# PoseLib/PoseLib

Measured on AMD Instinct MI355X. Metric: scored RANSAC hypotheses/sec (P3P@5k corrs, 5pt@5k corrs), higher is better.
Workload: dtype f64; 1 GPU; p3p_5000; correspondences=5000, problems_in_flight_per_gpu=128, distinct_scenes=64

## Files before the change

poselib_amd/csrc/kernels.hip:

```cpp
#include "pl_kernels.h"
#include "pl_global.h"
#include "pl_lm_chain.inc"
#include "pl_device.h"
#include <atomic>
#include "pl_prefilter.h"
#include <cstdlib>
#include "pl_sampler.h"
#include "pl_solver_h4.h"
#include "pl_solver_p3p.h"
#include "pl_solver_p5lp_radial.h"
#include "pl_solver_rel.h"

namespace pl {

typedef const float __attribute__((address_space(4))) *uniform_f32_ptr;
typedef const double __attribute__((address_space(4))) *uniform_f64_ptr;
typedef const uint32_t __attribute__((address_space(4))) *uniform_u32_ptr;
__device__ __forceinline__ uniform_f32_ptr as_uniform(const float *p) { return (uniform_f32_ptr)(uintptr_t)p; }
__device__ __forceinline__ uniform_f64_ptr as_uniform(const double *p) { return (uniform_f64_ptr)(uintptr_t)p; }
__device__ __forceinline__ uniform_u32_ptr as_uniform(const uint32_t *p) { return (uniform_u32_ptr)(uintptr_t)p; }

__device__ __forceinline__ double wave_sum(double v) {
#pragma unroll
    for (int off = 32; off > 0; off >>= 1)
// ... 840 lines not shown
                                                   const uint32_t *__restrict__ num_hyp_ptr, uint32_t hyp_capacity, double thr2,
                                                   const PrefilterArgs &pf, uint32_t *__restrict__ part_count,
                                                   double *__restrict__ part_score, uint32_t slice, uint32_t chunk,
                                                   uint32_t nslices) {
    constexpr int kWaves = kQueueThreads / 64;
    constexpr int ND = 5, P = kRadialP, NPW = kRadialChunk;
    __shared__ double s_pts[ND][NPW];
    __shared__ uint16_t s_queue[kWaves][kQueueCap];
    __shared__ double s_acc_s[kWaves][64];
    __shared__ uint32_t s_acc_c[kWaves][64];
    constexpr int kInlierCap = 128;
    __shared__ double s_inl_v[kWaves][kInlierCap];
    __shared__ uint16_t s_inl_g[kWaves][kInlierCap];
    __shared__ uint32_t s_next_unit;
    const int lane = threadIdx.x & 63;
    const int wave = __builtin_amdgcn_readfirstlane((int)(threadIdx.x >> 6));

    float pf32[P][ND];
    float bnd[P][2];
    uint64_t vmask[P];
    const float thrp = pf_radial1d_thr(pf.thr);
#pragma unroll
    for (int p = 0; p < P; ++p) {
        const uint32_t i = chunk * NPW + p * 64 + lane;
        const bool valid = i < pts.n;
        const uint32_t ic = valid ? i : 0u;
        vmask[p] = __builtin_amdgcn_ballot_w64(valid);
        double x[ND];
        load_point<EST_RAD1D>(pts, ic, x);
        if (wave == p) {
#pragma unroll
            for (int d = 0; d < ND; ++d)
                s_pts[d][p * 64 + lane] = x[d];
        }
        pf_radial1d_point(x, pf.thr, pf32[p], bnd[p]);
    }
    if (threadIdx.x == 0)
        s_next_unit = 0;
    __syncthreads();

    const uint32_t H = *as_uniform(num_hyp_ptr);
    const uniform_f32_ptr sh = as_uniform(shadow);
    uint16_t *const queue = s_queue[wave];
    double *const acc_s = s_acc_s[wave];
    uint32_t *const acc_c = s_acc_c[wave];
    double *const inl_v = s_inl_v[wave];
    uint16_t *const inl_g = s_inl_g[wave];

    const uint32_t waves_per_chunk = nslices * kWaves;
    auto request_ticket = [&]() -> uint32_t {
        uint32_t t = 0;
        if (lane == 0) {
            const uint32_t k = atomicAdd(&s_next_unit, 1u);
            t = slice * kWaves + (k % kWaves) + (k / kWaves) * waves_per_chunk;
        }
        return t;
    };
    uint32_t ticket = (uint32_t)__builtin_amdgcn_readfirstlane((int)request_ticket());
    uint32_t kb, gn;
    while (unit_of_ticket(ticket, H, waves_per_chunk, kb, gn)) {
        const uint32_t pending = request_ticket();
        acc_s[lane] = 0.0;
        acc_c[lane] = 0;
        uint32_t qhead = 0, qtail = 0;
        uint32_t ihead = 0, itail = 0;

        auto add_inliers = [&](uint32_t n) {
            __builtin_amdgcn_fence(__ATOMIC_ACQ_REL, "wavefront");
            const bool act = (uint32_t)lane < n;
            const uint32_t at = (ihead + lane) & (kInlierCap - 1);
            const uint32_t g = act ? (uint32_t)inl_g[at] : 0x7fu;
            const double v = act ? inl_v[at] : 0.0;
            const uint64_t actmask = __builtin_amdgcn_ballot_w64(act);
            const uint32_t g0 = (uint32_t)__builtin_amdgcn_readfirstlane((int)g);
            if (!__builtin_amdgcn_ballot_w64(act && g != g0)) {
                const double tot = wave_sum_dpp(v);
                if (lane == 0) {
                    acc_s[g0] += tot;
                    acc_c[g0] += (uint32_t)__popcll(actmask);
                }
            } else {
                add_run_totals(v, actmask, g, act, lane, acc_s, acc_c);
            }
            ihead += n;
        };

        auto drain = [&](uint32_t n) {
            __builtin_amdgcn_fence(__ATOMIC_ACQ_REL, "wavefront");
            const bool act = (uint32_t)lane < n;
            const uint32_t e = act ? (uint32_t)queue[(qhead + lane) & (kQueueCap - 1)] : 0xffffu;
            const uint32_t g = e >> 9, pi = act ? (e & 0x1ffu) : 0u;
            double x[ND];
#pragma unroll
            for (int d = 0; d < ND; ++d)
                x[d] = s_pts[d][pi];
            const double *Mp = compact64 + (size_t)(kb + (act ? g : 0u)) * kModelDoubles;
            double M[kModelDoubles];
#pragma unroll
            for (int i = 0; i < kModelDoubles; ++i)
                M[i] = Mp[i];
            double r2;
            const bool in = radial1d_inlier(M, x[0], x[1], x[2], x[3], x[4], thr2, r2) && act;
            const uint64_t inmask = __builtin_amdgcn_ballot_w64(in);
            if (inmask) {
                const uint32_t below = __builtin_amdgcn_mbcnt_hi((uint32_t)(inmask >> 32), __builtin_amdgcn_mbcnt_lo((uint32_t)inmask, 0u));
                if (in) {
                    inl_v[(itail + below) & (kInlierCap - 1)] = r2;
                    inl_g[(itail + below) & (kInlierCap - 1)] = (uint16_t)g;
                }
                itail += (uint32_t)__popcll(inmask);
                if (itail - ihead >= 64u)
                    add_inliers(64u);
            }
            qhead += n;
        };

        auto step = [&](const float(&r)[15], uint32_t g) {
            if ((r[0] != r[0]) | (r[1] != r[1]) | (r[2] != r[2]) | (r[3] != r[3]) | (r[4] != r[4]) | (r[5] != r[5]) | (r[9] != r[9]) | (r[10] != r[10]))
                return;
            uint64_t m[P];
            uint64_t any = 0;
            if (!pf.enabled || !(r[14] < __builtin_huge_valf())) {
#pragma unroll
                for (int p = 0; p < P; ++p)
                    m[p] = vmask[p], any |= m[p];
            } else {
#pragma unroll
                for (int p = 0; p < P; ++p) {
                    m[p] = vmask[p] & ~__builtin_amdgcn_ballot_w64(pf_radial1d_outlier(r, thrp, pf32[p], bnd[p]));
                    any |= m[p];
                }
            }
            if (any) {
#pragma unroll
                for (int p = 0; p < P; ++p) {
                    if (m[p]) {
                        const uint32_t below = __builtin_amdgcn_mbcnt_hi((uint32_t)(m[p] >> 32),
                                                                         __builtin_amdgcn_mbcnt_lo((uint32_t)m[p], 0u));
                        if ((m[p] >> lane) & 1u)
                            queue[(qtail + below) & (kQueueCap - 1)] = (uint16_t)((g << 9) | (uint32_t)(p * 64 + lane));
                        qtail += (uint32_t)__popcll(m[p]);
                    }
                }
                while (qtail - qhead >= 64u)
                    drain(64u);
            }
        };
        auto fetch = [&](float(&r)[15], uint32_t g) {
            const uniform_f32_ptr sp = sh + (size_t)(kb + g) * 16;
#pragma unroll
            for (int i = 0; i < 15; ++i)
                r[i] = sp[i];
        };

        float ra[15], rb[15];
        fetch(ra, 0);
        for (uint32_t g = 0; g < gn; g += 2) {
            const bool two = g + 1 < gn;
            if (two)
                fetch(rb, g + 1);
            step(ra, g);
            if (two) {
                if (g + 2 < gn)
                    fetch(ra, g + 2);
                step(rb, g + 1);
            }
        }
        while (qtail != qhead)
            drain(min(64u, qtail - qhead));
        if (itail != ihead)
            add_inliers(itail - ihead);
        __builtin_amdgcn_fence(__ATOMIC_ACQ_REL, "wavefront");
        if ((uint32_t)lane < gn) {
            const size_t o = (size_t)chunk * hyp_capacity + kb + lane;
            part_score[o] = acc_s[lane];
            part_count[o] = acc_c[lane];
        }
        ticket = (uint32_t)__builtin_amdgcn_readfirstlane((int)pending);
    }
}
__global__ __launch_bounds__(kQueueThreads) void k_score_radial1d(PointSet pts, const float *__restrict__ shadow,
                                                                  const double *__restrict__ compact64,
                                                                  const uint32_t *__restrict__ num_hyp_ptr, uint32_t hyp_capacity,
                                                                  double thr2, PrefilterArgs pf, uint32_t *__restrict__ part_count,
                                                                  double *__restrict__ part_score) {
    score_radial1d_body(pts, shadow, compact64, num_hyp_ptr, hyp_capacity, thr2, pf, part_count, part_score, blockIdx.x, blockIdx.y,
                       gridDim.x);
}

typedef _Float16 half4_t __attribute__((ext_vector_type(4)));
typedef _Float16 half8_t __attribute__((ext_vector_type(8)));
typedef float float16_t __attribute__((ext_vector_type(16)));
constexpr int kMfmaThreads = 512;

__device__ __forceinline__ bool slice_chunk_of_workgroup(uint32_t slices, uint32_t chunks, uint32_t &slice, uint32_t &chunk) {
    const uint32_t T = slices * chunks, L = blockIdx.x + gridDim.x * blockIdx.y;
    if (L >= T)
        return false;
    const uint32_t x = L & 7u, p = x * (T >> 3) + min(x, T & 7u) + (L >> 3);
    slice = p / chunks;
    chunk = p - slice * chunks;
    return true;
}

constexpr int kMfmaQueueCap = 1024;
template <int EST>
__device__ __forceinline__ void mfma_drain(const uint16_t *queue, uint32_t first, uint32_t n0, uint32_t n1, const double *pts, int npw,
                                       const double *__restrict__ models, uint32_t unit_slots, double thr2, double *acc_s,
                                       uint32_t *acc_c) {
    const int lane = threadIdx.x & 63;
    struct Batch {
        uint32_t g;
        bool act;
        double x[EST == EST_ABS ? 5 : 4];
        double M[kModelDoubles];
    };
    auto fetch = [&](uint32_t n, uint32_t at, Batch &b) {
        b.act = (uint32_t)lane < n;
        const uint32_t e = b.act ? (uint32_t)queue[(at + lane) & (kMfmaQueueCap - 1)] : 0xffffu;
        const uint32_t pi = b.act ? (e & 0x1ffu) : 0u;
        b.g = e >> 9;
#pragma unroll
        for (int d = 0; d < (EST == EST_ABS ? 5 : 4); ++d)
            b.x[d] = pts[d * npw + pi];
        const uint32_t slot_g = (uint32_t)__shfl((int)unit_slots, (int)(b.act ? b.g : 0u), 64);
        const double *Mp = models + (size_t)slot_g * kModelStride;
#pragma unroll
        for (int i = 0; i < kModelDoubles; ++i)
            b.M[i] = Mp[i];
    };
    auto finish = [&](const Batch &b) {
        double r2;
        const bool in = eval_point<EST>(b.M, b.x, thr2, r2) && b.act;
        const double v = in ? r2 : 0.0;
        const uint64_t inmask = __builtin_amdgcn_ballot_w64(in);
        const uint32_t g0 = (uint32_t)__builtin_amdgcn_readfirstlane((int)b.g);
        if (inmask && !__builtin_amdgcn_ballot_w64(b.act && b.g != g0)) {
            const double tot = wave_sum_dpp(v);
            if (lane == 0) {
                acc_s[g0] += tot;
                acc_c[g0] += (uint32_t)__popcll(inmask);
            }
        } else if (inmask) {
            add_run_totals(v, inmask, b.g, b.act, lane, acc_s, acc_c);
        }
    };
    __builtin_amdgcn_fence(__ATOMIC_ACQ_REL, "wavefront");
    Batch b0, b1;
    fetch(n0, first, b0);
    if (n1) {
        fetch(n1, first + n0, b1);
        finish(b0);
        finish(b1);
    } else {
        finish(b0);
    }
}

template <int PG>
__device__ __forceinline__ void abs16_tile_bits(const half8_t (&Aop)[kAbs16Dirs], const uint4 (&s_b)[1 + kAbs16Dirs][PG][32], int col, int half,
                                                uint32_t (&out)[16]) {
#pragma unroll
    for (int v = 0; v < 16; ++v)
        out[v] = 0u;
    const float16_t kZero = {0, 0, 0, 0, 0, 0, 0, 0, 0, 0, 0, 0, 0, 0, 0, 0};
    auto products = [&](int g, float16_t &D0, float16_t &D1, float16_t &D2) {
        half8_t Bop[kAbs16Dirs];
#pragma unroll
        for (int d = 0; d < kAbs16Dirs; ++d) {
            const uint4 braw = s_b[half ? 1 + d : 0][g][col];
            __builtin_memcpy(&Bop[d], &braw, 16);
        }
        D0 = __builtin_amdgcn_mfma_f32_32x32x16_f16(Aop[0], Bop[0], kZero, 0, 0, 0);
        D1 = __builtin_amdgcn_mfma_f32_32x32x16_f16(Aop[1], Bop[1], kZero, 0, 0, 0);
        D2 = __builtin_amdgcn_mfma_f32_32x32x16_f16(Aop[2], Bop[2], kZero, 0, 0, 0);
    };
    float16_t D0, D1, D2;
    products(0, D0, D1, D2);
#pragma unroll 16
    for (int g = 1; g < PG; ++g) {
        uint32_t T[16];
#pragma unroll
        for (int v = 0; v < 16; ++v)
            T[v] = __float_as_uint(D0[v]) | __float_as_uint(D1[v]) | __float_as_uint(D2[v]);
        products(g, D0, D1, D2);
#pragma unroll
        for (int v = 0; v < 16; ++v)
            out[v] = __builtin_amdgcn_alignbit(out[v], T[v], 31);
        __builtin_amdgcn_sched_group_barrier(0x002, 16, 0);
        __builtin_amdgcn_sched_group_barrier(0x100, 3, 0);
        __builtin_amdgcn_sched_group_barrier(0x002, 4, 0);
        __builtin_amdgcn_sched_group_barrier(0x008, 1, 0);
        __builtin_amdgcn_sched_group_barrier(0x002, 4, 0);
        __builtin_amdgcn_sched_group_barrier(0x008, 1, 0);
        __builtin_amdgcn_sched_group_barrier(0x002, 4, 0);
        __builtin_amdgcn_sched_group_barrier(0x008, 1, 0);
        __builtin_amdgcn_sched_group_barrier(0x002, 4, 0);
    }
#pragma unroll
    for (int v = 0; v < 16; ++v) {
        const uint32_t sg = __float_as_uint(D0[v]) | __float_as_uint(D1[v]) | __float_as_uint(D2[v]);
        out[v] = __builtin_amdgcn_alignbit(out[v], sg, 31);
    }
}

constexpr int kScoreAll = 0, kScoreLead = 1, kScoreSel = 2, kScoreCount = 3, kScoreCountAll = 4;
template <int PG, int MODE = kScoreAll>
__device__ __forceinline__ void score_mfma_body(const PointSet &pts, const uint4 *__restrict__ shadow16,
                                                const uint4 *__restrict__ points16,
                                                const double *__restrict__ models, const uint32_t *__restrict__ slots,
                                                const uint32_t *__restrict__ num_hyp_ptr, uint32_t hyp_capacity,
                                                double thr2, uint32_t *__restrict__ part_count,
                                                double *__restrict__ part_score, uint32_t slice, uint32_t chunk,
                                                uint32_t nslices, const uint32_t *__restrict__ sel = nullptr,
                                                uint32_t lead = 0) {
    constexpr int kWaves = kMfmaThreads / 64;
    constexpr int NPW = 32 * PG;
    __shared__ double s_pts[5][NPW];
    __shared__ uint16_t s_queue[kWaves][kMfmaQueueCap];
    __shared__ double s_acc_s[kWaves][64];
    __shared__ uint32_t s_acc_c[kWaves][64];
    __shared__ uint32_t s_next_unit;
    __shared__ uint4 s_b[1 + kAbs16Dirs][PG][32];
    const int lane = threadIdx.x & 63;
    const int wave = __builtin_amdgcn_readfirstlane((int)(threadIdx.x >> 6));
    const int col = lane & 31, half = lane >> 5;

    const uint32_t H = MODE == kScoreLead ? min(*as_uniform(num_hyp_ptr), lead) : *as_uniform(num_hyp_ptr);
    const uint32_t waves_per_chunk = nslices * kWaves;
    {
        uint32_t kb0, gn0;
        if (!unit_of_ticket<32u>(slice * kWaves, H, waves_per_chunk, kb0, gn0))
            return;
    }

    uint32_t validbits = 0;
#pragma unroll
    for (int g = 0; g < PG; ++g)
        validbits |= (chunk * NPW + g * 32 + col < pts.n) ? (1u << (PG - 1 - g)) : 0u;
    const uint4 *const prow = points16 + (size_t)chunk * NPW * 4;
    for (uint32_t j = threadIdx.x; j < (uint32_t)NPW; j += kMfmaThreads) {
        const uint32_t i = chunk * NPW + j;
        const uint32_t ic = i < pts.n ? i : 0u;
#pragma unroll
        for (int d = 0; d < 5; ++d)
            s_pts[d][j] = pts.a[d][ic];
#pragma unroll
        for (int r = 0; r < 1 + kAbs16Dirs; ++r)
            s_b[r][j >> 5][j & 31] = prow[(size_t)j * 4 + r];
    }
    if (threadIdx.x == 0)
        s_next_unit = 0;
    __syncthreads();

    uint16_t *const queue = s_queue[wave];
    double *const acc_s = s_acc_s[wave];
    uint32_t *const acc_c = s_acc_c[wave];
    auto request_ticket = [&]() -> uint32_t {
        uint32_t t = 0;
        if (lane == 0) {
            const uint32_t k = atomicAdd(&s_next_unit, 1u);
            t = slice * kWaves + (k % kWaves) + (k / kWaves) * waves_per_chunk;
        }
        return t;
    };
    uint32_t ticket = (uint32_t)__builtin_amdgcn_readfirstlane((int)request_ticket());
    uint32_t kb, gn;
    while (unit_of_ticket<32u>(ticket, H, waves_per_chunk, kb, gn)) {
        const uint32_t pending = request_ticket();
        uint32_t unit_pos = 0;
        if constexpr (MODE == kScoreSel)
            unit_pos = sel ? sel[kb + min((uint32_t)lane, gn - 1u)] : kb + min((uint32_t)lane, gn - 1u);
        const uint32_t unit_slots = slots[MODE == kScoreSel ? unit_pos : kb + min((uint32_t)lane, gn - 1u)];
        acc_s[lane] = 0.0;
        acc_c[lane] = 0;
        uint32_t qhead = 0, qtail = 0;

        auto drain_pair = [&](uint32_t n2) {
            mfma_drain<EST_ABS>(queue, qhead, 64u, n2, &s_pts[0][0], NPW, models, unit_slots, thr2, acc_s, acc_c);
            qhead += 64u + n2;
        };
        auto drain = [&](uint32_t n) {
            mfma_drain<EST_ABS>(queue, qhead, n, 0u, &s_pts[0][0], NPW, models, unit_slots, thr2, acc_s, acc_c);
            qhead += n;
        };

        const uint32_t ngroups32 = (gn + 31u) / 32u;
        auto load_a = [&](uint32_t hg, uint4 (&A)[kAbs16Dirs]) {
            const uint4 *row = shadow16 + (size_t)(kb + 32u * hg + (uint32_t)col) * 4;
            if constexpr (MODE == kScoreSel)
                row = shadow16 + (size_t)(uint32_t)__shfl((int)unit_pos, (int)(32u * hg + (uint32_t)col), 64) * 4;
#pragma unroll
            for (int d = 0; d < kAbs16Dirs; ++d)
                A[d] = row[half ? 3 : d];
        };
        uint4 Araw[kAbs16Dirs];
        load_a(0, Araw);
        for (uint32_t hg = 0; hg < ngroups32; ++hg) {
            half8_t Aop[kAbs16Dirs];
#pragma unroll
            for (int d = 0; d < kAbs16Dirs; ++d)
                __builtin_memcpy(&Aop[d], &Araw[d], 16);
            if (hg + 1 < ngroups32)
                load_a(hg + 1, Araw);
            uint32_t out[16];
            abs16_tile_bits<PG>(Aop, s_b, col, half, out);
            const bool partial_group = hg * 32u + 32u > gn;
            auto expand_round = [&](int v, bool check_slot) {
                const uint32_t slot = hg * 32u + 8u * (uint32_t)(v >> 2) + 4u * (uint32_t)half + (uint32_t)(v & 3);
                uint32_t bits = ~out[v] & validbits;
                if (check_slot && slot >= gn)
                    bits = 0u;
                const uint64_t anyb = __builtin_amdgcn_ballot_w64(bits != 0u);
                if (anyb) {
                    const uint32_t cnt = (uint32_t)__popc(bits);
                    if (!__builtin_amdgcn_ballot_w64(cnt > 1u)) {
                        const uint32_t below = __builtin_amdgcn_mbcnt_hi((uint32_t)(anyb >> 32), __builtin_amdgcn_mbcnt_lo((uint32_t)anyb, 0u));
                        if (bits) {
                            const uint32_t g = (uint32_t)(PG - 1 - (31 - __clz((int)bits)));
                            queue[(qtail + below) & (kMfmaQueueCap - 1)] = (uint16_t)((slot << 9) | (g * 32u + (uint32_t)col));
                        }
                        qtail += (uint32_t)__popcll(anyb);
                    } else {
                        const uint32_t incl = wave_scan_u32(cnt);
                        const uint32_t total = (uint32_t)__builtin_amdgcn_readlane((int)incl, 63);
                        uint32_t pos = qtail + incl - cnt;
                        uint32_t rest = bits;
                        while (rest) {
                            const int hi = 31 - __clz((int)rest);
                            rest &= ~(1u << hi);
                            const uint32_t g = (uint32_t)(PG - 1 - hi);
                            queue[pos & (kMfmaQueueCap - 1)] = (uint16_t)((slot << 9) | (g * 32u + (uint32_t)col));
                            ++pos;
                        }
                        qtail += total;
                    }
                    while (qtail - qhead >= 128u)
                        drain_pair(64u);
                }
            };
            if (partial_group) {
#pragma unroll
                for (int v = 0; v < 16; ++v)
                    expand_round(v, true);
            } else {
#pragma unroll
                for (int v = 0; v < 16; ++v)
                    expand_round(v, false);
            }
        }
        if (qtail - qhead > 64u)
            drain_pair(qtail - qhead - 64u);
        else if (qtail != qhead)
            drain(qtail - qhead);
        __builtin_amdgcn_fence(__ATOMIC_ACQ_REL, "wavefront");
        if ((uint32_t)lane < gn) {
            const size_t o = MODE == kScoreSel ? (size_t)chunk * hyp_capacity + unit_pos : (size_t)chunk * hyp_capacity + kb + lane;
            part_score[o] = acc_s[lane];
            part_count[o] = acc_c[lane];
        }
        ticket = (uint32_t)__builtin_amdgcn_readfirstlane((int)pending);
    }
}

template <int PG>
__device__ __forceinline__ void score_count_body(uint32_t n_points, const uint4 *__restrict__ shadow16, const uint4 *__restrict__ points16,
                                                 const uint32_t *__restrict__ num_hyp_ptr, uint32_t hyp_capacity,
                                                 uint32_t *__restrict__ survivors, uint32_t slice, uint32_t chunk, uint32_t nslices,
                                                 uint32_t first) {
    constexpr int kWaves = kMfmaThreads / 64;
    constexpr int NPW = 32 * PG;
    __shared__ uint4 s_b[1 + kAbs16Dirs][PG][32];
    __shared__ uint32_t s_cnt[kWaves][64];
    __shared__ uint32_t s_next_unit;
    const int lane = threadIdx.x & 63;
    const int wave = __builtin_amdgcn_readfirstlane((int)(threadIdx.x >> 6));
    const int col = lane & 31, half = lane >> 5;
    const uint32_t Hall = *as_uniform(num_hyp_ptr);
    if (Hall <= first)
        return;
    const uint32_t H = Hall - first;
    const uint32_t waves_per_chunk = nslices * kWaves;
    {
        uint32_t kb0, gn0;
        if (!unit_of_ticket<32u>(slice * kWaves, H, waves_per_chunk, kb0, gn0))
            return;
    }
    uint32_t validbits = 0;
#pragma unroll
    for (int g = 0; g < PG; ++g)
        validbits |= (chunk * NPW + g * 32 + col < n_points) ? (1u << (PG - 1 - g)) : 0u;
    const uint4 *const prow = points16 + (size_t)chunk * NPW * 4;
    for (uint32_t j = threadIdx.x; j < (uint32_t)NPW; j += kMfmaThreads) {
#pragma unroll
        for (int r = 0; r < 1 + kAbs16Dirs; ++r)
            s_b[r][j >> 5][j & 31] = prow[(size_t)j * 4 + r];
    }
    if (threadIdx.x == 0)
        s_next_unit = 0;
    __syncthreads();

    uint32_t *const cnt = s_cnt[wave];
    auto request_ticket = [&]() -> uint32_t {
        uint32_t t = 0;
        if (lane == 0) {
            const uint32_t k = atomicAdd(&s_next_unit, 1u);
            t = slice * kWaves + (k % kWaves) + (k / kWaves) * waves_per_chunk;
        }
        return t;
    };
    uint32_t ticket = (uint32_t)__builtin_amdgcn_readfirstlane((int)request_ticket());
    uint32_t kb, gn;
    while (unit_of_ticket<32u>(ticket, H, waves_per_chunk, kb, gn)) {
        const uint32_t pending = request_ticket();
        const uint32_t ngroups32 = (gn + 31u) / 32u;
        auto load_a = [&](uint32_t hg, uint4 (&A)[kAbs16Dirs]) {
            const uint4 *row = shadow16 + (size_t)min(first + kb + 32u * hg + (uint32_t)col, Hall - 1u) * 4;
#pragma unroll
            for (int d = 0; d < kAbs16Dirs; ++d)
                A[d] = row[half ? 3 : d];
        };
        uint4 Araw[kAbs16Dirs];
        load_a(0, Araw);
        for (uint32_t hg = 0; hg < ngroups32; ++hg) {
            half8_t Aop[kAbs16Dirs];
#pragma unroll
            for (int d = 0; d < kAbs16Dirs; ++d)
                __builtin_memcpy(&Aop[d], &Araw[d], 16);
            if (hg + 1 < ngroups32)
                load_a(hg + 1, Araw);
            uint32_t out[16];
            abs16_tile_bits<PG>(Aop, s_b, col, half, out);
            uint32_t pk[6] = {0u, 0u, 0u, 0u, 0u, 0u};
#pragma unroll
            for (int v = 0; v < 16; ++v)
                pk[v / 3] += (uint32_t)__popc(~out[v] & validbits) << (10 * (v % 3));
#pragma unroll
            for (int j = 0; j < 6; ++j) {
                uint32_t s = pk[j];
                s += dpp_shift_u32<0x111>(s);
                s += dpp_shift_u32<0x112>(s);
                s += dpp_shift_u32<0x114>(s);
                s += dpp_shift_u32<0x118>(s);
                s += dpp_shift_u32<0x142, 0xa>(s);
                pk[j] = s;
            }
            if (col == 31) {
#pragma unroll
                for (int v = 0; v < 16; ++v)
                    cnt[hg * 32u + 8u * (uint32_t)(v >> 2) + 4u * (uint32_t)half + (uint32_t)(v & 3)] = (pk[v / 3] >> (10 * (v % 3))) & 0x3ffu;
            }
        }
        __builtin_amdgcn_fence(__ATOMIC_ACQ_REL, "wavefront");
        if ((uint32_t)lane < gn)
            survivors[(size_t)chunk * hyp_capacity + first + kb + lane] = cnt[lane];
        __builtin_amdgcn_fence(__ATOMIC_ACQ_REL, "wavefront");
        ticket = (uint32_t)__builtin_amdgcn_readfirstlane((int)pending);
    }
}

template <int PG>
__global__ __launch_bounds__(kMfmaThreads) __attribute__((amdgpu_waves_per_eu(4, 8))) void k_score_mfma(PointSet pts, const uint4 *__restrict__ shadow16,
                                                               const uint4 *__restrict__ points16,
                                                               const double *__restrict__ models,
                                                               const uint32_t *__restrict__ slots,
                                                               const uint32_t *__restrict__ num_hyp_ptr,
                                                               uint32_t hyp_capacity, double thr2,
                                                               uint32_t *__restrict__ part_count,
                                                               double *__restrict__ part_score,
                                                               uint32_t *__restrict__ tickets) {
    (void)tickets;
    uint32_t slice, chunk;
    slice_chunk_of_workgroup(gridDim.x, gridDim.y, slice, chunk);
    score_mfma_body<PG>(pts, shadow16, points16, models, slots, num_hyp_ptr, hyp_capacity, thr2, part_count, part_score, slice,
                        chunk, gridDim.x);
}
template <int PG>
__global__ __launch_bounds__(kMfmaThreads) __attribute__((amdgpu_waves_per_eu(4, 8))) void k_score_mfma_g(const GroupArgs *ga) {
    const GroupArgs &g = ga[blockIdx.z];
    uint32_t slice, chunk;
    if (!g.active || !g.use_mfma || !slice_chunk_of_workgroup(g.slices, g.chunks, slice, chunk))
        return;
    const ScoreArgs a = globalised(g.score);
    score_mfma_body<PG>(a.pts, static_cast<const uint4 *>(a.shadow16), static_cast<const uint4 *>(a.points16), a.models, a.slots,
                        a.num_hyp, a.hyp_capacity, a.thr2, a.part_count, a.part_score, slice, chunk, g.slices);
}
template <int MODE> __host__ __device__ constexpr uint32_t pruned_slices(uint32_t slices) {
    return MODE == kScoreLead ? (slices < 2u ? slices : 2u) : MODE == kScoreSel ? (slices + 3u) / 4u : slices;
}
template <int PG, int MODE> __device__ __forceinline__ void score_mfma_pruned(const ScoreArgs &a, uint32_t slice, uint32_t chunk, uint32_t nslices) {
    static_assert(MODE == kScoreLead || MODE == kScoreSel || MODE == kScoreCount || MODE == kScoreCountAll, "the plain launch is k_score_mfma's");
    const PruneArgs &pr = a.prune;
    if (!pr.st && MODE != kScoreSel)
        return;
    if constexpr (MODE == kScoreCountAll) {
        score_count_body<PG>(a.pts.n, static_cast<const uint4 *>(a.shadow16), static_cast<const uint4 *>(a.points16), a.num_hyp,
                             a.hyp_capacity, a.part_count, slice, chunk, nslices, 0u);
    } else if constexpr (MODE == kScoreCount) {
        const uint32_t cstar = *as_uniform(&pr.st->cstar);
        if (cstar >= pr.chunks || chunk >= cstar)
            return;
        score_count_body<PG>(a.pts.n, static_cast<const uint4 *>(a.shadow16), static_cast<const uint4 *>(a.points16), a.num_hyp,
                             a.hyp_capacity, a.part_count, slice, chunk, nslices, pr.lead);
    } else {
        const uint32_t *len = MODE == kScoreSel && pr.st ? &pr.st->sel_len : a.num_hyp;
        score_mfma_body<PG, MODE>(a.pts, static_cast<const uint4 *>(a.shadow16), static_cast<const uint4 *>(a.points16), a.models, a.slots,
                                  len, a.hyp_capacity, a.thr2, a.part_count, a.part_score, slice, chunk, nslices, pr.st ? pr.sel : nullptr,
                                  pr.lead);
    }
}
template <int PG, int MODE>
__global__ __launch_bounds__(kMfmaThreads) __attribute__((amdgpu_waves_per_eu(4, 8))) void k_score_mfma_pr(ScoreArgs a) {
    uint32_t slice, chunk;
    slice_chunk_of_workgroup(gridDim.x, gridDim.y, slice, chunk);
    score_mfma_pruned<PG, MODE>(a, slice, chunk, gridDim.x);
}
template <int PG, int MODE>
__global__ __launch_bounds__(kMfmaThreads) __attribute__((amdgpu_waves_per_eu(4, 8))) void k_score_mfma_pr_g(const GroupArgs *ga) {
    const GroupArgs &g = ga[blockIdx.z];
    uint32_t slice, chunk;
    const uint32_t ns = pruned_slices<MODE>(g.slices);
    if (!g.active || !g.use_mfma || !slice_chunk_of_workgroup(ns, g.chunks, slice, chunk))
        return;
    score_mfma_pruned<PG, MODE>(globalised(g.score), slice, chunk, ns);
}

__device__ __forceinline__ void prune_lead_body(const ScoreArgs &a) {
    __shared__ uint32_t wmax[4];
    __shared__ double wmin[4];
    const PruneArgs &pr = a.prune;
    const uint32_t n = min(*a.num_hyp, pr.lead), N = a.pts.n;
    uint32_t bmax = 0;
    double bmin = 1.7976931348623157e308;
    for (uint32_t p = threadIdx.x; p < n; p += 256) {
        uint32_t c = 0;
        double s = 0.0;
        for (uint32_t ch = 0; ch < pr.chunks; ++ch) {
            c += a.part_count[(size_t)ch * a.hyp_capacity + p];
            s += a.part_score[(size_t)ch * a.hyp_capacity + p];
        }
        bmax = max(bmax, c);
        bmin = fmin(bmin, s + (double)(N - c) * a.thr2);
    }
#pragma unroll
    for (int off = 32; off > 0; off >>= 1) {
        bmax = max(bmax, (uint32_t)__shfl_xor(bmax, off, 64));
        bmin = fmin(bmin, __shfl_xor(bmin, off, 64));
    }
    if ((threadIdx.x & 63) == 0) {
        wmax[threadIdx.x >> 6] = bmax;
        wmin[threadIdx.x >> 6] = bmin;
    }
    __syncthreads();
    if (threadIdx.x == 0) {
        uint32_t lmax = pr.init_max;
        double lmin = pr.init_min;
        for (int w = 0; w < 4; ++w) {
            lmax = max(lmax, wmax[w]);
            lmin = fmin(lmin, wmin[w]);
        }
        const double need = fmax(lmin / a.thr2, (double)(N - min(lmax, N))) + (double)kPruneMargin;
        uint32_t cstar = pr.chunks;
        if (need < (double)N)
            cstar = (uint32_t)ceil(need / (double)pr.chunk_points);
        pr.st->lead_max = lmax;
        pr.st->lead_min = lmin;
        pr.st->cstar = max(1u, min(cstar, pr.chunks));
        pr.st->sel_len = 0;
        pr.st->pad = 0;
    }
}
__global__ __launch_bounds__(256) void k_prune_lead(ScoreArgs a) { prune_lead_body(a); }
__global__ __launch_bounds__(256) void k_prune_lead_g(const GroupArgs *ga) {
    const GroupArgs &g = ga[blockIdx.z];
    if (!g.active || !g.use_mfma || !g.score.prune.st)
        return;
    prune_lead_body(globalised(g.score));
}

__device__ __forceinline__ bool prune_rule(uint32_t cs, double sum, uint32_t S, uint32_t N, double thr2, const PruneState &st) {
    return cs + (N - S) <= st.lead_max && sum + (double)(S - cs) * thr2 > st.lead_min * (1.0 + kPruneScoreMargin);
}
__device__ __forceinline__ uint32_t prune_keeps(const ScoreArgs &a, uint32_t p, uint32_t H, uint32_t cstar) {
    const PruneArgs &pr = a.prune;
    if (p >= H)
        return 0u;
    if (p < pr.lead || cstar >= pr.chunks)
        return 1u;
    const uint32_t N = a.pts.n, S = min(cstar * pr.chunk_points, N);
    uint32_t cs = 0;
    for (uint32_t ch = 0; ch < cstar; ++ch)
        cs += a.part_count[(size_t)ch * a.hyp_capacity + p];
    return prune_rule(cs, 0.0, S, N, a.thr2, *pr.st) ? 0u : 1u;
}
__global__ __launch_bounds__(256) void k_prune_label(ScoreArgs a) {
    const PruneArgs &pr = a.prune;
    const uint32_t H = *a.num_hyp, cstar = pr.st->cstar, p = blockIdx.x * 256u + threadIdx.x;
    if (p >= H || p < pr.lead || cstar >= pr.chunks || pr.kept[p] != kKept)
        return;
    const uint32_t N = a.pts.n, S = min(cstar * pr.chunk_points, N);
    uint32_t cs = 0;
    double sum = 0.0;
    for (uint32_t ch = 0; ch < cstar; ++ch) {
        cs += a.part_count[(size_t)ch * a.hyp_capacity + p];
        sum += a.part_score[(size_t)ch * a.hyp_capacity + p];
    }
    if (prune_rule(cs, sum, S, N, a.thr2, *pr.st))
        pr.kept[p] = kPrunedExact;
}
__device__ __forceinline__ void prune_flags_body(const ScoreArgs &a) {
    __shared__ uint32_t wt[16];
    const PruneArgs &pr = a.prune;
    const uint32_t H = *a.num_hyp, cstar = pr.st->cstar;
    if (blockIdx.x * 1024u >= H)
        return;
    const uint32_t p = blockIdx.x * 1024u + threadIdx.x;
    const uint32_t keep = prune_keeps(a, p, H, cstar);
    if (p < H)
        pr.kept[p] = (uint8_t)keep;
    const uint32_t tot = wave_sum_u32(keep);
    if ((threadIdx.x & 63) == 0)
        wt[threadIdx.x >> 6] = tot;
    __syncthreads();
    if (threadIdx.x == 0) {
        uint32_t t = 0;
        for (int w = 0; w < 16; ++w)
            t += wt[w];
        pr.blk_kept[blockIdx.x] = t;
    }
}
__device__ __forceinline__ void prune_list_body(const ScoreArgs &a) {
    __shared__ uint32_t wt[16], wb[16];
    const PruneArgs &pr = a.prune;
    const uint32_t H = *a.num_hyp;
    if (blockIdx.x * 1024u >= H)
        return;
    const int lane = threadIdx.x & 63, wave = threadIdx.x >> 6;
    uint32_t before = 0;
    for (uint32_t j = threadIdx.x; j < blockIdx.x; j += 1024u)
        before += pr.blk_kept[j];
    before = wave_sum_u32(before);
    const uint32_t p = blockIdx.x * 1024u + threadIdx.x;
    const uint32_t keep = p < H ? (uint32_t)pr.kept[p] : 0u;
    const uint32_t inc = wave_scan_u32(keep);
    if (lane == 63)
        wt[wave] = inc;
    if (lane == 0)
        wb[wave] = before;
    __syncthreads();
    uint32_t at = inc - keep;
    for (int w = 0; w < 16; ++w)
        at += wb[w] + (w < wave ? wt[w] : 0u);
    if (keep)
        pr.sel[at] = p;
    if (p == H - 1u)
        pr.st->sel_len = at + keep;
}
__global__ __launch_bounds__(1024) void k_prune_flags(ScoreArgs a) { prune_flags_body(a); }
__global__ __launch_bounds__(1024) void k_prune_list(ScoreArgs a) { prune_list_body(a); }
__global__ __launch_bounds__(1024) void k_prune_flags_g(const GroupArgs *ga) {
    const GroupArgs &g = ga[blockIdx.z];
    if (!g.active || !g.use_mfma || !g.score.prune.st)
        return;
    prune_flags_body(globalised(g.score));
}
__global__ __launch_bounds__(1024) void k_prune_list_g(const GroupArgs *ga) {
    const GroupArgs &g = ga[blockIdx.z];
    if (!g.active || !g.use_mfma || !g.score.prune.st)
        return;
    prune_list_body(globalised(g.score));
}

constexpr int kBoundThreads = 512;
constexpr uint32_t kBoundGroups = 16;
template <int P> __device__ __forceinline__ void score_bound_body(const ScoreArgs &a, uint32_t wg, uint32_t nwg) {
    constexpr int kWaves = kBoundThreads / 64;
    constexpr uint32_t NPW = 64u * P;
    __shared__ uint32_t s_c[kWaves][64];
    __shared__ uint64_t s_q[kWaves][64];
    __shared__ uint32_t s_und[64];
    __shared__ uint32_t s_nund;
    const PruneArgs &pr = a.prune;
    if (!pr.st || !pr.bound || *as_uniform(&pr.st->cstar) >= pr.chunks)
        return;
    const uint32_t first = min(*as_uniform(a.num_hyp), pr.lead), len = *as_uniform(&pr.st->sel_len);
    if (len <= first || (uint64_t)wg * 64u >= len - first)
        return;
    const int lane = threadIdx.x & 63;
    const int wave = __builtin_amdgcn_readfirstlane((int)(threadIdx.x >> 6));
    const PrefilterArgs pf = a.pf;
    const uint32_t chunks = pr.chunks;
    const bool resident = chunks <= (uint32_t)kWaves;
    float x[P], y[P], X[P], Y[P], Z[P], fw[P];
    bool valid[P];
    uint64_t vmask[P];
    auto load_chunk = [&](uint32_t chunk) {
#pragma unroll
        for (int p = 0; p < P; ++p) {
            const uint32_t i = chunk * NPW + (uint32_t)p * 64u + (uint32_t)lane;
            valid[p] = i < a.pts.n;
            vmask[p] = __builtin_amdgcn_ballot_w64(valid[p]);
            const uint32_t ic = valid[p] ? i : 0u;
            const double Xd = a.pts.a[2][ic], Yd = a.pts.a[3][ic], Zd = a.pts.a[4][ic];
            x[p] = (float)a.pts.a[0][ic], y[p] = (float)a.pts.a[1][ic];
            X[p] = (float)Xd, Y[p] = (float)Yd, Z[p] = (float)Zd;
            fw[p] = pf_point_abs(Xd, Yd, Zd, pf.gx);
        }
    };
    load_chunk(min((uint32_t)wave, chunks - 1u));
    const uint32_t lead_max = pr.st->lead_max;
    const double beat = pr.st->lead_min * (1.0 + kPruneScoreMargin);
    auto decide = [&](uint32_t pos) -> bool {
        uint32_t c = 0;
        uint64_t q = 0;
#pragma unroll
        for (int w = 0; w < kWaves; ++w) {
            c += s_c[w][lane];
            q += s_q[w][lane];
        }
        const double qd = (double)q * 9.5367431640625e-07;
        double s_lb = a.thr2 * qd;
        if (fma(a.thr2, qd, -s_lb) < 0.0)
            s_lb = __longlong_as_double(__double_as_longlong(s_lb) - 1);
        const bool keep = !(c <= lead_max && s_lb > beat);
        if (!keep)
            pr.kept[pos] = kDropped;
        if (pr.bnd_count)
            pr.bnd_count[pos] = c, pr.bnd_score[pos] = s_lb;
        return keep;
    };
    const uint32_t nent = len - first;
    for (uint32_t u = wg; (uint64_t)u * 64u < nent; u += nwg) {
        const uint32_t e = first + u * 64u + (uint32_t)lane;
        const uint32_t pos = pr.sel[min(e, len - 1u)];
        const float4 *sh = reinterpret_cast<const float4 *>(a.models + (size_t)a.slots[pos] * kModelStride + kShadowOff);
        float4 rv[4];
#pragma unroll
        for (int k = 0; k < 4; ++k)
            rv[k] = sh[k];
        const uint32_t n = min(64u, nent - u * 64u);
        auto model_of_lane = [&](uint32_t j, float (&r)[16]) {
#pragma unroll
            for (int k = 0; k < 4; ++k) {
                r[4 * k + 0] = __builtin_bit_cast(float, __builtin_amdgcn_readlane(__builtin_bit_cast(int, rv[k].x), (int)j));
                r[4 * k + 1] = __builtin_bit_cast(float, __builtin_amdgcn_readlane(__builtin_bit_cast(int, rv[k].y), (int)j));
                r[4 * k + 2] = __builtin_bit_cast(float, __builtin_amdgcn_readlane(__builtin_bit_cast(int, rv[k].z), (int)j));
                r[4 * k + 3] = __builtin_bit_cast(float, __builtin_amdgcn_readlane(__builtin_bit_cast(int, rv[k].w), (int)j));
            }
        };
        uint32_t my_c = 0;
        uint64_t my_q = 0;
        for (uint32_t ch = (uint32_t)wave; ch < chunks; ch += (uint32_t)kWaves) {
            if (!resident)
                load_chunk(ch);
            for (uint32_t j = 0; j < n; ++j) {
                float r[16];
                model_of_lane(j, r);
                const float gt = pf_abs_bound_slack(r, pf.gx);
                uint32_t c = 0, q = 0;
// ... 2581 lines not shown
```

Baseline: 1.309 billion hypotheses/s.

## Count inliers per hypothesis lane directly from MFMA outputs, dropping DPP reduction

The count-scoring kernel now reads the MFMA result along its hypothesis axis, so each lane accumulates its own hypothesis's inlier count by packing sign bits into words and popcounting them. The two wave halves are combined with a single permlane32 swap, and each lane writes its result straight to global memory. This removes the per-point validity mask, the packed DPP prefix reductions, the LDS staging buffer and its fences. Padded points are handled by subtracting a per-chunk pad count, which assumes padded entries always test as inliers. That assumption is a correctness risk if the padding data differs.

```diff
diff --git a/poselib_amd/csrc/kernels.hip b/poselib_amd/csrc/kernels.hip
--- a/poselib_amd/csrc/kernels.hip
+++ b/poselib_amd/csrc/kernels.hip
@@ -1166,6 +1166,57 @@
         const uint32_t sg = __float_as_uint(D0[v]) | __float_as_uint(D1[v]) | __float_as_uint(D2[v]);
         out[v] = __builtin_amdgcn_alignbit(out[v], sg, 31);
     }
+}
+
+template <int PG>
+__device__ __forceinline__ uint32_t abs16_tile_count_t(const half8_t (&Aop)[kAbs16Dirs], const uint4 (&s_b)[1 + kAbs16Dirs][PG][32], int col,
+                                                       int half) {
+    static_assert(PG % 2 == 0, "a word holds the 32 pairs of two point groups");
+    const float16_t kZero = {0, 0, 0, 0, 0, 0, 0, 0, 0, 0, 0, 0, 0, 0, 0, 0};
+    auto products = [&](int g, float16_t &D0, float16_t &D1, float16_t &D2) {
+        half8_t Bop[kAbs16Dirs];
+#pragma unroll
+        for (int d = 0; d < kAbs16Dirs; ++d) {
+            const uint4 braw = s_b[half ? 1 + d : 0][g][col];
+            __builtin_memcpy(&Bop[d], &braw, 16);
+        }
+        D0 = __builtin_amdgcn_mfma_f32_32x32x16_f16(Bop[0], Aop[0], kZero, 0, 0, 0);
+        D1 = __builtin_amdgcn_mfma_f32_32x32x16_f16(Bop[1], Aop[1], kZero, 0, 0, 0);
+        D2 = __builtin_amdgcn_mfma_f32_32x32x16_f16(Bop[2], Aop[2], kZero, 0, 0, 0);
+    };
+    uint32_t word = 0u, n = 0u;
+    float16_t D0, D1, D2;
+    products(0, D0, D1, D2);
+#pragma unroll 16
+    for (int g = 1; g < PG; ++g) {
+        uint32_t T[16];
+#pragma unroll
+        for (int v = 0; v < 16; ++v)
+            T[v] = __float_as_uint(D0[v]) | __float_as_uint(D1[v]) | __float_as_uint(D2[v]);
+        products(g, D0, D1, D2);
+#pragma unroll
+        for (int v = 0; v < 16; ++v)
+            word = __builtin_amdgcn_alignbit(word, T[v], 31);
+        if ((g - 1) % 2)
+            n += (uint32_t)__popc(word);
+        __builtin_amdgcn_sched_group_barrier(0x002, 16, 0);
+        __builtin_amdgcn_sched_group_barrier(0x100, 3, 0);
+        __builtin_amdgcn_sched_group_barrier(0x002, 4, 0);
+        __builtin_amdgcn_sched_group_barrier(0x008, 1, 0);
+        __builtin_amdgcn_sched_group_barrier(0x002, 4, 0);
+        __builtin_amdgcn_sched_group_barrier(0x008, 1, 0);
+        __builtin_amdgcn_sched_group_barrier(0x002, 4, 0);
+        __builtin_amdgcn_sched_group_barrier(0x008, 1, 0);
+        __builtin_amdgcn_sched_group_barrier(0x002, 4, 0);
+        __builtin_amdgcn_sched_barrier(0);
+    }
+#pragma unroll
+    for (int v = 0; v < 16; ++v) {
+        const uint32_t sg = __float_as_uint(D0[v]) | __float_as_uint(D1[v]) | __float_as_uint(D2[v]);
+        word = __builtin_amdgcn_alignbit(word, sg, 31);
+    }
+    n += (uint32_t)__popc(word);
+    return 16u * PG - n;
 }
 
 constexpr int kScoreAll = 0, kScoreLead = 1, kScoreSel = 2, kScoreCount = 3, kScoreCountAll = 4;
@@ -1335,10 +1386,8 @@
     constexpr int kWaves = kMfmaThreads / 64;
     constexpr int NPW = 32 * PG;
     __shared__ uint4 s_b[1 + kAbs16Dirs][PG][32];
-    __shared__ uint32_t s_cnt[kWaves][64];
     __shared__ uint32_t s_next_unit;
     const int lane = threadIdx.x & 63;
-    const int wave = __builtin_amdgcn_readfirstlane((int)(threadIdx.x >> 6));
     const int col = lane & 31, half = lane >> 5;
     const uint32_t Hall = *as_uniform(num_hyp_ptr);
     if (Hall <= first)
@@ -1350,10 +1399,7 @@
         if (!unit_of_ticket<32u>(slice * kWaves, H, waves_per_chunk, kb0, gn0))
             return;
     }
-    uint32_t validbits = 0;
-#pragma unroll
-    for (int g = 0; g < PG; ++g)
-        validbits |= (chunk * NPW + g * 32 + col < n_points) ? (1u << (PG - 1 - g)) : 0u;
+    const uint32_t pad = chunk * NPW + NPW > n_points ? chunk * NPW + NPW - n_points : 0u;
     const uint4 *const prow = points16 + (size_t)chunk * NPW * 4;
     for (uint32_t j = threadIdx.x; j < (uint32_t)NPW; j += kMfmaThreads) {
 #pragma unroll
@@ -1364,7 +1410,6 @@
         s_next_unit = 0;
     __syncthreads();
 
-    uint32_t *const cnt = s_cnt[wave];
     auto request_ticket = [&]() -> uint32_t {
         uint32_t t = 0;
         if (lane == 0) {
@@ -1393,32 +1438,14 @@
                 __builtin_memcpy(&Aop[d], &Araw[d], 16);
             if (hg + 1 < ngroups32)
                 load_a(hg + 1, Araw);
-            uint32_t out[16];
-            abs16_tile_bits<PG>(Aop, s_b, col, half, out);
-            uint32_t pk[6] = {0u, 0u, 0u, 0u, 0u, 0u};
-#pragma unroll
-            for (int v = 0; v < 16; ++v)
-                pk[v / 3] += (uint32_t)__popc(~out[v] & validbits) << (10 * (v % 3));
-#pragma unroll
-            for (int j = 0; j < 6; ++j) {
-                uint32_t s = pk[j];
-                s += dpp_shift_u32<0x111>(s);
-                s += dpp_shift_u32<0x112>(s);
-                s += dpp_shift_u32<0x114>(s);
-                s += dpp_shift_u32<0x118>(s);
-                s += dpp_shift_u32<0x142, 0xa>(s);
-                pk[j] = s;
-            }
-            if (col == 31) {
-#pragma unroll
-                for (int v = 0; v < 16; ++v)
-                    cnt[hg * 32u + 8u * (uint32_t)(v >> 2) + 4u * (uint32_t)half + (uint32_t)(v & 3)] = (pk[v / 3] >> (10 * (v % 3))) & 0x3ffu;
-            }
-        }
-        __builtin_amdgcn_fence(__ATOMIC_ACQ_REL, "wavefront");
-        if ((uint32_t)lane < gn)
-            survivors[(size_t)chunk * hyp_capacity + first + kb + lane] = cnt[lane];
-        __builtin_amdgcn_fence(__ATOMIC_ACQ_REL, "wavefront");
+            const uint32_t mine = abs16_tile_count_t<PG>(Aop, s_b, col, half);
+            const auto both = __builtin_amdgcn_permlane32_swap(mine, mine, false, false);
+            uint32_t total = both[0] + both[1];
+            if (pad)
+                total = max(total, pad) - pad;
+            if (half == 0 && 32u * hg + (uint32_t)col < gn)
+                survivors[(size_t)chunk * hyp_capacity + first + kb + 32u * hg + (uint32_t)col] = total;
+        }
         ticket = (uint32_t)__builtin_amdgcn_readfirstlane((int)pending);
     }
 }
```

Result: faster. 1.376 billion hypotheses/s (median of 6 runs) (+5.2%).
